# QizhiPei/FABind

Measured on AMD Instinct MI355X. Metric: complexes/sec fwd+bwd (1500p/40l nodes), full IaBNet on the whole graph (pocket model + 4-layer complex model + distance-map head on all nodes / pairs) with the pocket-cls + pocket-centre + coord + distmap + distmap-by-coords + distill losses (BASELINE configs[2] read literally), higher is better.
Workload: dtype bf16

## Files before the change

fabind_amd/_lib.py:

```python
import ctypes
import os

import torch

from . import config as _cfg

_HERE = os.path.dirname(os.path.abspath(__file__))
LIB_PATH = _cfg.knob("FABIND_LIB") or os.path.join(_HERE, "libfabind_hip.so")

ABI_VERSION = 19
DT_F32, DT_BF16 = 0, 1
ACT_NONE, ACT_SILU, ACT_RELU, ACT_SIGMOID, ACT_STORED_DERIV = 0, 1, 2, 3, 4
GEMM_FAM_NT_F32, GEMM_FAM_NT_F32_BF16, GEMM_FAM_NT_BF16, GEMM_FAM_GLDS, GEMM_FAM_PIPE, GEMM_FAM_X3, GEMM_FAM_X3_PRO, GEMM_FAM_PERSIST = range(8)

_vp, _i, _f, _l = ctypes.c_void_p, ctypes.c_int, ctypes.c_float, ctypes.c_long


class GemmArgs(ctypes.Structure):
    _fields_ = [(n, _vp) for n in ("A", "A2", "W", "C", "bias", "R", "r_index", "dotvec", "dot_out", "aux", "groups", "C2")] + \
               [(n, _i) for n in ("M", "N", "K", "K1", "lda", "lda2", "ldw", "ldc", "ldr", "ldaux", "dot_ld",
                                  "a_dtype", "w_dtype", "c_dtype", "aux_dtype", "act_pro", "act_epi", "dact_epi",
                                  "accumulate", "store_preact", "n_groups", "max_m", "max_n", "groups_ext", "epi_fast", "k_splits")] + \
               [("alpha", _f), ("p_drop", _f), ("drop_seed", ctypes.c_uint)] + \
               [(n, _vp) for n in ("row_mu", "row_rs", "col_c", "C16")] + [("ldc16", _i), ("split3", _i), ("r_dtype", _i), ("c2_bf16", _i)]
# ... 105 lines not shown
    "fabind_rowdot_bwd": [_vp, _i, _vp, _i, _vp, _i, _i, _i, _vp, _vp, _vp, _i, _vp],
    "fabind_edge_geom_bwd": [_vp, _vp, _vp, _vp, _vp, _vp, _vp, _vp, _vp, _vp, _i, _i, _i, _vp, _vp, _vp, _vp],
    "fabind_gcl_pre_bwd": [_vp, _i, _i, _vp, _vp, _i, _vp, _vp, _vp, _i, _vp],
    "fabind_gather_dact": [_vp, _i, _vp, _vp, _i, _i, _vp, _i, _i, _i, _vp],
    "fabind_coord_update_bwd": [_vp, _vp, _vp, _i, _i, _f, _vp, _vp, _vp, _vp],
    "fabind_cross_attn_bwd": [_vp, _i, _vp, _i, _vp, _i, _i, _i, _vp, _i, _i, _i, _f, _vp, _vp, _vp, _vp, _vp, _vp, _vp,
                              _vp, _vp, _vp],
    "fabind_pair_bias_cat": [_vp, _i, _vp, _i, _i, _i, _vp, _i, _vp, _i, _vp, _vp, _i, _vp, _i, _vp, _vp],
    "fabind_batched_transpose_pad": [_vp, _i, _vp, _i, _i, _i, _i, _vp, _vp],
    "fabind_node_chain_fwd": [_vp, _i, _vp, _i, _vp, _vp, _vp, _vp, _vp, _vp, _i, _i, _vp, _i, _vp, _i, _vp, _i, _i, _i, _vp],
    "fabind_node_chain_x3_fwd": [_vp, _i, _vp, _i, _vp, _vp, _vp, _vp, _vp, _vp, _vp, _vp, _vp, _vp, _i, _i, _vp, _i, _vp, _i, _vp, _i, _vp, _i, _vp, _i,
                                 _i, _i, _vp],
    "fabind_rows_hadamard_bwd": [_vp, _i, _i, _vp, _i, _i, _vp, _vp, _vp, _i, _vp, _i, _vp],
    "fabind_pair_hadamard_bwd_grid": [_vp, _i, _i, _vp, _i, _i, _vp, _vp, _vp, _vp, _i, _vp, _i, _vp],
    "fabind_pair_hadamard_bwd_rows": [_vp, _i, _i, _vp, _i, _i, _vp, _i, _i, _vp, _vp, _vp, _vp, _i, _vp, _i, _vp, _i, _vp],
    "fabind_pair_hadamard_bwd": [_vp, _i, _i, _vp, _vp, _i, _i, _vp, _vp, _i, _i, _vp, _vp, _i, _vp, _vp, _i, _vp, _vp, _i,
                                 _vp],
    "fabind_inter_attn_bwd": [_vp, _i, _vp, _i, _i, _vp, _vp, _vp, _vp, _vp, _vp, _vp, _vp, _vp, _vp, _vp, _vp, _f, _i,
                              _vp, _vp, _vp, _vp, _vp, _vp, _vp, _vp, _vp, _vp, _i, _vp],
    "fabind_inter_attn_bwd_rows": [_vp, _i, _vp, _i, _i, _vp, _vp, _vp, _vp, _vp, _vp, _vp, _vp, _vp, _vp, _vp, _vp, _f, _i,
                                   _vp, _vp, _vp, _vp, _vp, _vp, _vp, _vp, _vp, _vp, _i, _vp, _i, _i, _vp],
    "fabind_las_step_bwd": [_vp, _vp, _vp, _vp, _vp, _vp, _vp, _vp, _i, _i, _f, _f, _vp, _vp, _vp],
    "fabind_pair_bias_bwd": [_vp, _i, _vp, _i, _i, _vp, _vp, _i, _i, _i, _vp, _vp, _vp, _vp, _vp],
    "fabind_pair_bias_btcat": [_vp, _i, _vp, _vp, _vp, _i, _i, _i, _vp, _i, _i, _vp],
    "fabind_pair_bias_finish": [_vp, _vp, _i, _i, _vp, _vp, _i, _vp, _vp, _l, _vp],
    "fabind_pack_frag_multi": [_vp, _vp, _i, _vp],
    "fabind_lower_bound": [_vp, _i, _vp, _i, _vp, _vp],
    "fabind_pocket_center_fwd": [_vp, _vp, _vp, _vp, _i, _i, _f, _i, _vp, _vp, _vp],
    "fabind_pocket_center_bwd": [_vp, _vp, _vp, _vp, _i, _i, _f, _vp, _vp, _vp, _vp, _vp],
    "fabind_pair_dist_fwd": [_vp, _i, _i, _vp, _vp, _f, _f, _f, _vp, _vp],
    "fabind_pair_dist_bwd": [_vp, _i, _i, _vp, _vp, _vp, _f, _f, _f, _vp, _vp, _vp],
    "fabind_block_hadamard_fwd": [_vp, _i, _i, _vp, _i, _vp, _i, _i, _vp, _i, _vp],
    "fabind_block_hadamard_bwd": [_vp, _i, _i, _vp, _i, _vp, _i, _vp, _i, _i, _vp, _i, _i, _vp, _vp, _i, _vp, _i, _vp],
    "fabind_loss_fwd": [_vp, _vp, _l, _vp, _vp, _vp, _l, _vp, _vp, _i, _vp, _l, _vp, _vp, _l, _f, _f, _f, _f, _f, _f, _vp, _vp, _vp, _vp, _vp, _vp],
    "fabind_loss_bwd": [_vp, _vp, _l, _vp, _vp, _vp, _l, _vp, _vp, _i, _l, _vp, _vp, _l, _f, _f, _f, _f, _f, _f, _vp, _vp, _vp,
                        _vp, _vp, _vp, _vp, _vp, _vp],
    "fabind_layernorm_fwd": [_vp, _vp, _vp, _f, _i, _i, _vp, _vp, _vp, _vp],
    "fabind_layernorm_bwd": [_vp, _vp, _vp, _vp, _vp, _i, _i, _vp, _vp, _vp, _vp],
}

_lib = None


def load():
    global _lib
    if _lib is not None:
        return _lib
    if not os.path.exists(LIB_PATH):
        raise RuntimeError(
            "fabind_amd: %s is missing -- build it with `python -m fabind_amd.build` (hipcc, gfx950). "
            "There is no CPU/eager fallback for the hot path." % LIB_PATH)
    lib = ctypes.CDLL(LIB_PATH)
    lib.fabind_last_error.restype = ctypes.c_char_p
    lib.fabind_abi_version.restype = ctypes.c_int
    got = lib.fabind_abi_version()
    if got != ABI_VERSION:
        raise RuntimeError("fabind_amd: %s has ABI version %d, this binding needs %d -- rebuild with `python -m fabind_amd.build`"
                           % (LIB_PATH, got, ABI_VERSION))
    lib.fabind_sizeof_args.argtypes, lib.fabind_sizeof_args.restype = [ctypes.c_int], ctypes.c_int
    lib.fabind_cross_attn_bwd_scratch.argtypes, lib.fabind_cross_attn_bwd_scratch.restype = [_i, _i, _i], ctypes.c_long
    lib.fabind_pair_bias_cat_parts.argtypes, lib.fabind_pair_bias_cat_parts.restype = [_i, _i], ctypes.c_long
    lib.fabind_cross_attn_fused_bwd_scratch.argtypes, lib.fabind_cross_attn_fused_bwd_scratch.restype = [_i, _i, _i, _i, _i], ctypes.c_long
    lib.fabind_cross_attn_fused_bwd_parts.argtypes, lib.fabind_cross_attn_fused_bwd_parts.restype = [_i, _i], ctypes.c_int
    lib.fabind_pair_bias_finish_parts.argtypes, lib.fabind_pair_bias_finish_parts.restype = [_i], ctypes.c_int
    lib.fabind_loss_blocks.argtypes, lib.fabind_loss_blocks.restype = [_l, _l, _l], ctypes.c_int
    for nm in ("fabind_pair_block_tile", "fabind_pair_block_chunk"):
# ... 58 lines not shown
```

fabind_amd/build.py:

```python
import os
import subprocess
import sys

HERE = os.path.dirname(os.path.abspath(__file__))
CSRC = os.path.join(HERE, "csrc")
INCLUDE = os.path.join(os.path.dirname(HERE), "include")
LIB = os.path.join(HERE, "libfabind_hip.so")
SOURCES = ["capi.hip", "gemm.hip", "graph.hip", "gcl.hip", "fused_edge.hip", "fused_edge_fwd2.hip", "fused_edge_fwd3.hip", "fused_edge_bwd3.hip", "fused_edge_bwd4.hip", "pair_fused.hip", "attn.hip", "inter_attn_rows.hip", "attn_mfma.hip", "norm.hip", "bwd.hip", "post_optim.hip", "node_chain.hip", "heads.hip", "symmetry.hip", "optim.hip", "ranking.hip"]
HIPCC = os.environ.get("HIPCC", "/opt/rocm/bin/hipcc")
FLAGS = ["--offload-arch=gfx950", "-O3", "-std=c++17", "-fPIC", "-Wno-comment", "-I" + INCLUDE, "-I" + CSRC]


def _stale(out, deps):
    if not os.path.exists(out):
        return True
    t = os.path.getmtime(out)
    return any(os.path.getmtime(d) > t for d in deps)


def build(force=False, verbose=True):
    objs = []
    hdrs = [os.path.join(CSRC, "common.h"), os.path.join(CSRC, "fused_common.h"), os.path.join(INCLUDE, "fabind_hip.h")]
    procs = []
    for src in SOURCES:
        sp = os.path.join(CSRC, src)
        if not os.path.exists(sp):
            raise RuntimeError("fabind_amd.build: source %s is missing" % sp)
        obj = os.path.join(CSRC, src.replace(".hip", ".o"))
        objs.append(obj)
        if force or _stale(obj, [sp] + hdrs):
            cmd = [HIPCC] + FLAGS + ["-c", sp, "-o", obj]
            if verbose:
                print(" ".join(cmd), flush=True)
            procs.append((src, subprocess.Popen(cmd)))
    for src, p in procs:
        if p.wait() != 0:
            raise RuntimeError("hipcc failed on " + src)
    if force or procs or _stale(LIB, objs):
        cmd = [HIPCC, "--offload-arch=gfx950", "-shared", "-fPIC", "-o", LIB] + objs
        if verbose:
            print(" ".join(cmd), flush=True)
        subprocess.check_call(cmd)
    return LIB


if __name__ == "__main__":
    build(force="--force" in sys.argv)
```

fabind_amd/csrc/heads.hip:

```cpp
#include "common.h"
#include "fabind_hip.h"

namespace {

constexpr int LOSS_THREADS = 256;
constexpr int LOSS_TERMS = 8;

__device__ __forceinline__ float agent_load(const float* p) { return __hip_atomic_load(p, __ATOMIC_RELAXED, __HIP_MEMORY_SCOPE_AGENT); }
__device__ __forceinline__ void agent_store(float* p, float v) { __hip_atomic_store(p, v, __ATOMIC_RELAXED, __HIP_MEMORY_SCOPE_AGENT); }

__device__ __forceinline__ float cls_target(const void* cls, int cls_dt, long i) {
    switch (cls_dt) {
        case 0: return ((const float*)cls)[i];
        case 1: return (float)((const long long*)cls)[i];
        case 2: return (float)((const int*)cls)[i];
        default: return (float)((const uint8_t*)cls)[i];
    }
}

__global__ __launch_bounds__(LOSS_THREADS) void loss_fwd_kernel(
    const float* __restrict__ coords, const float* __restrict__ coords_true, long n_coord, const float* __restrict__ y_pred,
    const float* __restrict__ y_by, const float* __restrict__ dis_map, long n_pair, const float* __restrict__ logits,
    const void* __restrict__ cls, int cls_dt, const uint8_t* __restrict__ mask, long n_cls, const float* __restrict__ center,
    const float* __restrict__ center_true, long n_center, float w_coord, float w_pair, float w_distill, float w_cls, float w_center,
    float delta, float* part, unsigned* ticket, float* out, float* loss_out, float* terms_out) {
    const long tid = (long)blockIdx.x * LOSS_THREADS + threadIdx.x, nthr = (long)gridDim.x * LOSS_THREADS;
    float acc[7] = {0.f, 0.f, 0.f, 0.f, 0.f, 0.f, 0.f};
    for (long i = tid; i < n_pair; i += nthr) {
        const float yp = y_pred[i], yb = y_by[i], dm = dis_map[i];
        const float a = yp - dm, b = yb - dm, c = yb - yp;
        acc[2] += a * a; acc[3] += b * b; acc[4] += c * c;
    }
    for (long i = tid; i < n_coord; i += nthr) {
        const float d = fabsf(coords[i] - coords_true[i]);
// ... 126 lines not shown
    const int lane = threadIdx.x & 63, wave = threadIdx.x >> 6;
#pragma unroll
    for (int k = 0; k < 4; ++k) {
        const float v = wave_sum(a[k]);
        if (lane == 0) sh[wave][k] = v;
    }
    __syncthreads();
    if (threadIdx.x == 0) {
        float t[4];
#pragma unroll
        for (int k = 0; k < 4; ++k) t[k] = ((sh[0][k] + sh[1][k]) + sh[2][k]) + sh[3][k];
        center[b * 3] = t[1] / t[0]; center[b * 3 + 1] = t[2] / t[0]; center[b * 3 + 2] = t[3] / t[0];
        wsum[b] = t[0];
    }
}

__global__ __launch_bounds__(256) void pocket_center_bwd_kernel(const float* __restrict__ logits, const uint8_t* __restrict__ mask,
                                                                const float* __restrict__ xyz, const float* __restrict__ noise,
                                                                int L, float inv_tau, const float* __restrict__ center,
                                                                const float* __restrict__ wsum, const float* __restrict__ dcenter,
                                                                long n, float* dlogits) {
    const long i = (long)blockIdx.x * 256 + threadIdx.x;
    if (i >= n) return;
    if (!mask[i]) { dlogits[i] = 0.f; return; }
    const int b = (int)(i / L);
    float ds;
    (void)pc_soft(logits[i], noise, i, inv_tau, &ds);
    const float dw = (dcenter[b * 3] * (xyz[i * 3] - center[b * 3]) + dcenter[b * 3 + 1] * (xyz[i * 3 + 1] - center[b * 3 + 1]) +
                      dcenter[b * 3 + 2] * (xyz[i * 3 + 2] - center[b * 3 + 2])) / wsum[b];
    dlogits[i] = dw * ds;
}


constexpr int PB_TP = 128;
constexpr int PB_CH = 20;

struct PairBlock { long pair_off; int P, C, p_row0, c_row0, tile0, pad; };

__device__ __forceinline__ int pb_find(const PairBlock* __restrict__ desc, int B, int tile) {
    int lo = 0, hi = B - 1;
    while (lo < hi) {
        const int mid = (lo + hi + 1) >> 1;
        if (desc[mid].tile0 <= tile) lo = mid; else hi = mid - 1;
    }
    return lo;
}

__global__ __launch_bounds__(256) void pair_dist_fwd_kernel(const PairBlock* __restrict__ desc, int B, const float* __restrict__ xp,
                                                            const float* __restrict__ xc, float scale, float lo, float hi, float* y) {
    const int b = pb_find(desc, B, blockIdx.x);
    const PairBlock d = desc[b];
    const int i0 = (blockIdx.x - d.tile0) * PB_TP, i1 = min(d.P, i0 + PB_TP);
    if (i0 >= d.P) return;
    const long n = (long)(i1 - i0) * d.C;
    for (long k = threadIdx.x; k < n; k += 256) {
        const int i = i0 + (int)(k / d.C), j = (int)(k % d.C);
        const float* a = xp + (size_t)(d.p_row0 + i) * 3;
        const float* c = xc + (size_t)(d.c_row0 + j) * 3;
        const float dx = a[0] - c[0], dy = a[1] - c[1], dz = a[2] - c[2];
        const float v = scale * sqrtf(dx * dx + dy * dy + dz * dz);
        y[d.pair_off + (long)i0 * d.C + k] = fminf(fmaxf(v, lo), hi);
    }
}

__global__ __launch_bounds__(256) void pair_dist_bwd_kernel(const PairBlock* __restrict__ desc, const float* __restrict__ xp,
                                                            const float* __restrict__ xc, const float* __restrict__ dy, float scale,
                                                            float lo, float hi, int max_C, float* part) {
    const int b = blockIdx.x, s = blockIdx.y;
    const PairBlock d = desc[b];
    __shared__ float sh[256][3];
    for (int j0 = 0; j0 < d.C; j0 += 256) {
        const int cw = min(256, d.C - j0);
        const int nl = 256 / cw, il = threadIdx.x / cw, j = j0 + threadIdx.x % cw;
        float ax = 0.f, ay = 0.f, az = 0.f;
        if (il < nl) {
            const float* c = xc + (size_t)(d.c_row0 + j) * 3;
            const float cx = c[0], cy = c[1], cz = c[2];
            for (int i = s + 8 * il; i < d.P; i += 8 * nl) {
                const float* a = xp + (size_t)(d.p_row0 + i) * 3;
// ... 79 lines not shown
                if (j < cw) *(float2*)(sm + ((size_t)il * PB_CH + j) * W + c2) = acc[j];
            __syncthreads();
            for (int k = threadIdx.x; k < cw * W; k += 256) {
                float v = 0.f;
                for (int l = 0; l < NL; ++l) v += sm[(size_t)l * PB_CH * W + k];
                po[k] = v;
            }
        }
    }
}
template <int W>
__global__ __launch_bounds__(256) void block_hadamard_fwd_kernel(const PairBlock* __restrict__ desc, int B, const float* __restrict__ tp,
                                                                 int ldtp, const float* __restrict__ tc, int ldtc, bf16_t* out, int ldo) {
    constexpr int CT = W / 8, RP = 256 / CT;
    const int b = pb_find(desc, B, blockIdx.x);
    const PairBlock d = desc[b];
    const int i0 = (blockIdx.x - d.tile0) * PB_TP, i1 = min(d.P, i0 + PB_TP);
    if (i0 >= d.P) return;
    const int ct = threadIdx.x % CT, rg = threadIdx.x / CT, c8 = ct * 8;
    for (int i = i0; i < i1; ++i) {
        const float4 p0 = *(const float4*)(tp + (size_t)(d.p_row0 + i) * ldtp + c8), p1 = *(const float4*)(tp + (size_t)(d.p_row0 + i) * ldtp + c8 + 4);
        bf16_t* orow = out + (size_t)(d.pair_off + (long)i * d.C) * ldo + c8;
        for (int j = rg; j < d.C; j += RP) {
            const float* c = tc + (size_t)(d.c_row0 + j) * ldtc + c8;
            const float4 q0 = *(const float4*)c, q1 = *(const float4*)(c + 4);
            typedef __attribute__((ext_vector_type(4))) unsigned int nc_u4;
            const nc_u4 v = {pack2_bf16(p0.x * q0.x, p0.y * q0.y), pack2_bf16(p0.z * q0.z, p0.w * q0.w),
                             pack2_bf16(p1.x * q1.x, p1.y * q1.y), pack2_bf16(p1.z * q1.z, p1.w * q1.w)};
            __builtin_nontemporal_store(v, (nc_u4*)(orow + (size_t)j * ldo));
        }
    }
}

__global__ __launch_bounds__(256) void block_hadamard_bwd_reduce_kernel(const PairBlock* __restrict__ desc, int B, const int* __restrict__ row_b,
                                                                        int W, int nchunk_max, const float* __restrict__ part, float* dtc,
                                                                        int lddc) {
    const int r = blockIdx.x, b = row_b[r];
    const PairBlock d = desc[b];
    const int j = r - d.c_row0, ch = j / PB_CH, jj = j % PB_CH;
    const int nt = (d.P + PB_TP - 1) / PB_TP;
    for (int c = threadIdx.x; c < W; c += 256) {
        float v = 0.f;
        for (int t = 0; t < nt; ++t) v += part[(((size_t)(d.tile0 + t) * nchunk_max + ch) * PB_CH + jj) * W + c];
        dtc[(size_t)r * lddc + c] = v;
    }
}

}

extern "C" int fabind_pair_block_tile(void) { return PB_TP; }
extern "C" int fabind_pair_block_chunk(void) { return PB_CH; }

extern "C" int fabind_pair_dist_fwd(const void* desc, int B, int n_tiles, const float* xp, const float* xc, float scale, float lo, float hi,
                                    float* y, hipStream_t stream) {
    if (B <= 0 || n_tiles <= 0) return 0;
    hipLaunchKernelGGL(pair_dist_fwd_kernel, dim3(n_tiles), dim3(256), 0, stream, (const PairBlock*)desc, B, xp, xc, scale, lo, hi, y);
    FB_CHECK_LAUNCH();
    return 0;
}
extern "C" int fabind_pair_dist_bwd(const void* desc, int B, int max_C, const float* xp, const float* xc, const float* dy, float scale,
                                    float lo, float hi, float* part, float* dxc, hipStream_t stream) {
    if (B <= 0) return 0;
    FB_REQUIRE(part && dxc && max_C > 0, "fabind_pair_dist_bwd: scratch [B][8][max_C][3] and the output are required");
    hipLaunchKernelGGL(pair_dist_bwd_kernel, dim3(B, 8), dim3(256), 0, stream, (const PairBlock*)desc, xp, xc, dy, scale, lo, hi, max_C, part);
    FB_CHECK_LAUNCH();
    hipLaunchKernelGGL(pair_dist_bwd_reduce_kernel, dim3(B), dim3(256), 0, stream, (const PairBlock*)desc, B, max_C, part, dxc);
    FB_CHECK_LAUNCH();
    return 0;
}
extern "C" int fabind_block_hadamard_fwd(const void* desc, int B, int n_tiles, const float* tp, int ldtp, const float* tc, int ldtc, int W,
                                         void* out, int ldo, hipStream_t stream) {
    FB_REQUIRE(W == 64 || W == 128 || W == 256 || W == 512, "fabind_block_hadamard_fwd: W in {64, 128, 256, 512}");
    FB_REQUIRE(ldtp % 4 == 0 && ldtc % 4 == 0 && ldo % 8 == 0 && ((((uintptr_t)tp | (uintptr_t)tc | (uintptr_t)out) & 15) == 0),
               "fabind_block_hadamard_fwd: 16-byte aligned rows");
    if (B <= 0 || n_tiles <= 0) return 0;
    const PairBlock* dd = (const PairBlock*)desc;
    bf16_t* o = (bf16_t*)out;
    if (W == 512) hipLaunchKernelGGL((block_hadamard_fwd_kernel<512>), dim3(n_tiles), dim3(256), 0, stream, dd, B, tp, ldtp, tc, ldtc, o, ldo);
    else if (W == 256) hipLaunchKernelGGL((block_hadamard_fwd_kernel<256>), dim3(n_tiles), dim3(256), 0, stream, dd, B, tp, ldtp, tc, ldtc, o, ldo);
    else if (W == 128) hipLaunchKernelGGL((block_hadamard_fwd_kernel<128>), dim3(n_tiles), dim3(256), 0, stream, dd, B, tp, ldtp, tc, ldtc, o, ldo);
// ... 90 lines not shown
```

fabind_amd/models/model.py:

```python
import random

import torch
import torch.nn as nn
import torch.nn.functional as F
from torch.nn import Linear

from .. import kernels as K
from .. import ops
from ..utils.utils import get_keepNode_tensor, gumbel_softmax_no_random
from .att_model import EfficientMCAttModel


class Transition_diff_out_dim(nn.Module):

    def __init__(self, embedding_channels=256, out_channels=256, n=4):
        super().__init__()
        self.layernorm = nn.LayerNorm(embedding_channels)
        self.linear1 = Linear(embedding_channels, n * embedding_channels)
        self.linear2 = Linear(n * embedding_channels, out_channels)
        torch.nn.init.xavier_uniform_(self.linear1.weight, gain=0.001)
        torch.nn.init.xavier_uniform_(self.linear2.weight, gain=0.001)

    def forward(self, z):
        shp = z.shape
# ... 252 lines not shown
        start = _offsets(reps)
        j = torch.arange(pi.shape[0], device=dev) - start[pi]
        ci = _offsets(ncnt)[pocket_batch][pi] + j
        kn = torch.stack([kcnt, ncnt]).tolist()
        return _Pairs(pi, ci, ops.PairBlocks(kn[0], kn[1], dev))

    def _complex_and_heads(self, data, g, plan=None):
        scale = self.coordinate_scale
        cb = data['compound'].batch
        if plan:
            Xn, Xl, cidx, pidx = plan['Xn'], plan['Xl'], plan['cidx'], plan['pidx']
        else:
            Xn = self.normalize_coord(g['X'].unsqueeze(-2)).float()
            Xl = self.normalize_coord(g['XL'].unsqueeze(-2)).float()
            seg1 = g['segment'].bool() if not g['segment'].is_floating_point() else g['segment'] > 0.5
            cidx = torch.nonzero(~seg1 & ~g['is_global']).squeeze(1)
            pidx = torch.nonzero(seg1 & ~g['is_global']).squeeze(1)
        Xo, Ho = self.complex_model(Xn, g['H'], batch_id=g['batch'], segment_id=g['segment'], mask=g['mask'],
                                    is_global=g['is_global'], compound_edge_index=g['c2c'], LAS_edge_index=g['LAS'],
                                    batched_complex_coord_LAS=Xl, LAS_mask=None)
        coords_n = ops.take_unique_rows(Xo, cidx).squeeze(-2)
        return Ho, cidx, pidx, coords_n

    def _dist_heads(self, data, g, Ho, cidx, pidx, coords_n):
        cb = data['compound'].batch
        pairs = g.get('pairs')
        if pairs is None:
            B = int(cb[-1].item()) + 1
            pairs = self._pair_lists(g['pocket_batch'], cb, torch.bincount(g['pocket_batch'], minlength=B), torch.bincount(cb, minlength=B))
        pi, ci = pairs
        ln = ops.layernorm(ops.take_unique_rows(Ho, torch.cat([pidx, cidx])), self.layernorm.weight, self.layernorm.bias, self.layernorm.eps)
        npk = pidx.shape[0]
        blocks = getattr(pairs, 'blocks', None)
        hd = ops.rows_hadamard(ln, pi, npk + ci, a_sorted=True, blocks=blocks, n_a=npk)
        wd = ops.mm_dtype()
        part = ops.linear_rowdot(hd, self.distmap_mlp[0].weight.to(wd), self.distmap_mlp[0].bias,
                                 self.distmap_mlp[2].weight[0].contiguous(), act_epi=K.ACT_RELU)
        y_pred = (part.sum(1) + self.distmap_mlp[2].bias).sigmoid() * 10
        xp = self.normalize_coord(g['pocket_xyz']).float()
        if blocks is not None and coords_n.is_cuda:
            y_by = ops.pair_dist(xp, coords_n, blocks, scale=self.coordinate_scale, lo=0.0, hi=10.0)
        else:
            y_by = self.unnormalize_coord((xp[pi] - ops.take_rows_few(coords_n, ci)).norm(dim=-1)).clamp(0, 10)
        return y_pred, y_by

    def forward(self, data, stage=1, train=False, plan=None):
        cb = data['compound'].batch
        if plan is not None:
            self._adopt_plan(plan, cb.device)
        if plan is not None:
            keep_idx = plan['keep_idx']
        else:
            keep_idx = torch.nonzero(data['pocket'].keepNode).squeeze(1) if (stage == 1 or self.pocket_pred_model.training) else None
        head = self._pocket_head(data, plan)
        training = self.pocket_pred_model.training
        center = self._soft_center(head['logits'], head['mask'], head['xyz'], noise=training)
        pocket_cls = torch.zeros_like(head['mask'], dtype=data.pocket_idx.dtype)
        pocket_cls[head['pb'], head['loc']] = data.pocket_idx
        if training:
            dist = torch.norm(data.coords_center - center, p=2, dim=-1).mean(dim=-1)
            final_stage = 2 if (dist < self.args.center_dist_threshold and random.random() < self.stage_prob) else 1
        else:
            final_stage = stage
        if final_stage == 2:
            c2 = center
            if self.args.local_eval or (self.args.train_pred_pocket_noise and train):
                c2 = center + self.args.train_pred_pocket_noise * (2 * torch.rand_like(center) - 1)
            g = self._stage2(data, head, c2)
        else:
            cx = data['complex']
# ... 63 lines not shown
```

fabind_amd/ops.py:

```python
import ctypes

import numpy as np
import torch

from . import config as _cfg
from . import kernels as K
from ._lib import GemmArgs, check, dt_code, load, ptr, stream


def act_dtype():
    return torch.float32 if _cfg.fp32_storage() else torch.bfloat16


mm_dtype = act_dtype


def needs_grad(*ts):
    return torch.is_grad_enabled() and any(torch.is_tensor(t) and t.requires_grad for t in ts)


_needs_grad = needs_grad


def _nchunk(rows):
# ... 1219 lines not shown
        check(load().fabind_pair_hadamard_bwd(ptr(dout), dt_code(dout.dtype), dout.stride(0), ptr(t), ptr(t), t.stride(0), W,
                                              None, None, 0, 0, ptr(ia), ptr(ib), ia.shape[0], ptr(dt_), ptr(dt_),
                                              dt_.stride(0), None, None, 0, stream()), "fabind_pair_hadamard_bwd")
        return dt_, None, None, None, None, None


def _rows_hadamard_csr(ia, ib, n, a_sorted=False):
    P = ia.shape[0]
    dev = ia.device
    ia64, ib64 = ia.long(), ib.long()
    pa = torch.arange(P, device=dev) if a_sorted else torch.argsort(ia64, stable=True)
    pb = torch.argsort(ib64, stable=True)
    one = torch.ones_like(ia64)
    ca = torch.zeros(n, dtype=torch.int64, device=dev).index_add_(0, ia64, one)
    cb_ = torch.zeros(n, dtype=torch.int64, device=dev).index_add_(0, ib64, one)
    rowptr = torch.zeros(n + 1, dtype=torch.int64, device=dev)
    rowptr[1:] = torch.cumsum(ca + cb_, 0)
    starts = rowptr[:-1]
    sa, sb = ia64[pa], ib64[pb]
    ar = torch.arange(P, device=dev)
    ra = ar - (torch.cumsum(ca, 0) - ca)[sa]
    rb = ar - (torch.cumsum(cb_, 0) - cb_)[sb]
    pair_idx = torch.empty(2 * P, dtype=torch.int32, device=dev)
    partner = torch.empty(2 * P, dtype=torch.int32, device=dev)
    posa, posb = starts[sa] + ra, starts[sb] + ca[sb] + rb
    pair_idx[posa], partner[posa] = pa.to(torch.int32), ib64[pa].to(torch.int32)
    pair_idx[posb], partner[posb] = pb.to(torch.int32), ia64[pb].to(torch.int32)
    return rowptr.to(torch.int32), pair_idx, partner


ROWS_HADAMARD_WALK = _cfg.knob("FABIND_ROWS_HADAMARD_WALK")


def _block_hadamard_fwd(t, bl, n_a):
    W = t.shape[1]
    if not (bl is not None and act_dtype() == torch.bfloat16 and t.dtype == torch.float32 and W in (64, 128, 256, 512) and t.stride(1) == 1
            and t.stride(0) % 4 == 0 and t.data_ptr() % 16 == 0 and n_a == bl.n_prows and t.shape[0] == bl.n_prows + bl.n_crows and n_a % 4 == 0):
        return None
    out = torch.empty((bl.n_pairs, W), dtype=torch.bfloat16, device=t.device)
    check(load().fabind_block_hadamard_fwd(bl.desc_ptr, bl.B, bl.n_tiles, ptr(t), t.stride(0), ptr(t[n_a:]), t.stride(0), W, ptr(out), W,
                                           stream()), "fabind_block_hadamard_fwd")
    return out


def rows_hadamard(t, idx_a, idx_b, a_sorted=False, blocks=None, n_a=0):
    ia, ib = idx_a.to(torch.int32).contiguous(), idx_b.to(torch.int32).contiguous()
    if _needs_grad(t):
        return _RowsHadamard.apply(t, ia, ib, a_sorted, blocks, n_a)
    fwd = _block_hadamard_fwd(t, blocks, n_a)
    if fwd is not None:
        return fwd
    dummy = t[:, :0]
    return K.pair_hadamard(t, t, dummy, dummy, ia, ib, act_dtype())


class _InterAttn(torch.autograd.Function):
    @staticmethod
    def forward(ctx, qkv, cv, h, x, d, rhohat, bias_part, w_rk, w_rv, wcr, w3, H, g, clampv, s_ext=None, Wc=None, bc=None, holder=None, Wc32=None):
        v_in = None
        if Wc is not None:
            c16 = getattr(qkv, "_fab_b16", None) if _cfg.get_precision() == "bf16" else None
            v_in = c16[1][:, 2 * H:] if (c16 is not None and c16[0] == qkv._version) else _mm_in(qkv[:, 2 * H:])
            if Wc32 is not None:
                cv, _ = K.gemm(qkv[:, 2 * H:], Wc32, bias=bc, force_x3=True)
            else:
                cv, _ = K.gemm(v_in, Wc, bias=bc)
        h16 = None
        if holder is not None:
            h16 = torch.empty((h.shape[0], H), dtype=torch.bfloat16, device=h.device)
            holder.append(h16)
        h_out, x_out, alpha, cvs = K.inter_attn_fwd(qkv, cv, H, h, x, d, rhohat, g.rp_int, g.col_int, g.red_idx,
                                                    bias_part, w_rk, w_rv, wcr, w3, clampv, s_ext, h16, deal=getattr(g, "int_deal", None))
        ctx.g, ctx.H, ctx.clampv, ctx.np = g, H, clampv, bias_part.shape[1]
        ctx.has_ext, ctx.has_cv = s_ext is not None, Wc is not None
        ctx.sink_h, ctx.Wct = _sink_of(h), (_stored_wt(Wc) if Wc is not None else None)
# ... 619 lines not shown
```

include/fabind_hip.h:

```cpp
#ifndef FABIND_HIP_H
#define FABIND_HIP_H

#include <stdint.h>

#ifdef __cplusplus
extern "C" {
#endif

#ifndef __HIP_PLATFORM_AMD__
typedef struct ihipStream_t* hipStream_t;
#endif

const char* fabind_last_error(void);
#define FABIND_ABI_VERSION 19
int fabind_abi_version(void);
int fabind_sizeof_args(int which);

typedef struct FabindGemmArgs {
    const void* A;
    const void* A2;
    const void* W;
    void* C;
    const float* bias;
    const void* R;
// ... 243 lines not shown
int fabind_las_step(const float* x, const float* x0, const int* las_i, const int* las_j, const int* las_off,
                    const int* node_off, const int* c_cnt, int B, int max_n, float step, float clampv, float* x_out,
                    unsigned char* pass_mask, hipStream_t stream);

int fabind_pocket_center_fwd(const float* logits, const uint8_t* mask, const float* xyz, const float* noise, int B, int L,
                             float tau, int hard, float* center, float* wsum, hipStream_t stream);
int fabind_pocket_center_bwd(const float* logits, const uint8_t* mask, const float* xyz, const float* noise, int B, int L,
                             float tau, const float* center, const float* wsum, const float* dcenter, float* dlogits,
                             hipStream_t stream);

int fabind_loss_blocks(long n_pair, long n_coord, long n_cls);
int fabind_loss_fwd(const float* coords, const float* coords_true, long n_coord, const float* y_pred, const float* y_by,
                    const float* dis_map, long n_pair, const float* logits, const void* cls, int cls_dt, const uint8_t* mask,
                    long n_cls, const float* center, const float* center_true, long n_center, float w_coord, float w_pair,
                    float w_distill, float w_cls, float w_center, float delta, float* part, unsigned* ticket, float* out,
                    float* loss_out, float* terms_out, hipStream_t stream);
int fabind_loss_bwd(const float* coords, const float* coords_true, long n_coord, const float* y_pred, const float* y_by,
                    const float* dis_map, long n_pair, const float* logits, const void* cls, int cls_dt, long n_cls,
                    const float* center, const float* center_true, long n_center, float w_coord, float w_pair, float w_distill,
                    float w_cls, float w_center, float delta, const float* fwd_out, const float* g_loss, const float* g_terms,
                    float* d_coords, float* d_y_pred, float* d_y_by, float* d_logits, float* d_center, hipStream_t stream);

int fabind_pair_block_tile(void);
int fabind_pair_block_chunk(void);
int fabind_pair_dist_fwd(const void* desc, int B, int n_tiles, const float* xp, const float* xc, float scale, float lo, float hi,
                         float* y, hipStream_t stream);
int fabind_pair_dist_bwd(const void* desc, int B, int max_C, const float* xp, const float* xc, const float* dy, float scale, float lo,
                         float hi, float* part, float* dxc, hipStream_t stream);
int fabind_block_hadamard_fwd(const void* desc, int B, int n_tiles, const float* tp, int ldtp, const float* tc, int ldtc, int W, void* out,
                              int ldo, hipStream_t stream);
int fabind_block_hadamard_bwd(const void* desc, int B, int n_tiles, const void* dout, int ldo, const float* tp, int ldtp,
                              const float* tc, int ldtc, int W, const int* row_b, int n_crows, int nchunk_max, float* part,
                              float* dtp, int lddp, float* dtc, int lddc, hipStream_t stream);

int fabind_select_rows(const float* x, const float* z, const uint8_t* mask, int n, int width, float* x_out,
                       hipStream_t stream);

int fabind_row_stats(const void* x, int x_dt, int ldx, float eps, int R, int C, float* mu, float* rs, hipStream_t stream);

int fabind_layernorm_rows(const void* x, int x_dt, int ldx, const float* w, const float* b, float eps, int R, int C, void* y,
                          int y_dt, int ldy, int pad_to, hipStream_t stream);
int fabind_edge_ln_concat(const float* h, int ldh, int H, const int* row, const int* col, const float* rhohat, const float* w,
                          const float* b, float eps, int E, void* y, int y_dt, int ldy, int pad_to, hipStream_t stream);

int fabind_edge_lnfold(const void* AB, int ldab, int Kp, int H, const int* row, const int* col, const float* rho,
                       const float* stat, float eps, const float* w_r, const float* c_r, const float* c_c, const float* dvec,
                       int E, void* out, float p_drop, unsigned seed, hipStream_t stream);
int fabind_edge_lnfold_bwd_blocks(int E);
int fabind_edge_lnfold_bwd(const void* AB, int ldab, int Kp, int H, const int* row, const int* col, const float* rho,
                           const float* stat, float eps, const float* w_r, const float* c_r, const float* c_c,
                           const void* out, const void* dout, int E, float p_drop, void* du, float* es,
                           float* drho, float* part, int n_blocks, hipStream_t stream);

int fabind_inter_coord_fold(const void* P, int ldp, int H, const int* col, const float* rho, const float* stat, float q_w,
                            float eps, const float* u, const float* d, const float* w3, int E, float* s_out, float p_drop,
                            unsigned seed, hipStream_t stream);
int fabind_layernorm_rows_bwd(const void* x, int x_dt, int ldx, const float* w, const void* dy, int dy_dt, int lddy, float eps,
                              int R, int C, void* dx, int dx_dt, int lddx, float* dw_part, float* db_part, int nblk, hipStream_t stream);
int fabind_edge_concat(const float* h, int ldh, int H, const int* row, const int* col, const float* rhohat, int E, void* y,
                       int y_dt, int ldy, int pad_to, hipStream_t stream);
int fabind_layernorm_fwd(const float* x, const float* w, const float* b, float eps, int R, int C, float* y, float* mean,
                         float* rstd, hipStream_t stream);
int fabind_layernorm_bwd(const float* x, const float* w, const float* dy, const float* mean, const float* rstd, int R,
                         int C, float* dx, float* dw_part, float* db_part, hipStream_t stream);

int fabind_add(const float* a, const float* b, float* out, long n, hipStream_t stream);
// ... 93 lines not shown
```

Measured before the change: 528.2.

## Fuse distance-map head backward: compute d(hadamard) in registers and reduce to row grads

```diff
diff --git a/fabind_amd/_lib.py b/fabind_amd/_lib.py
--- a/fabind_amd/_lib.py
+++ b/fabind_amd/_lib.py
@@ -161,6 +161,7 @@
     "fabind_pair_dist_bwd": [_vp, _i, _i, _vp, _vp, _vp, _f, _f, _f, _vp, _vp, _vp],
     "fabind_block_hadamard_fwd": [_vp, _i, _i, _vp, _i, _vp, _i, _i, _vp, _i, _vp],
     "fabind_block_hadamard_bwd": [_vp, _i, _i, _vp, _i, _vp, _i, _vp, _i, _i, _vp, _i, _i, _vp, _vp, _i, _vp, _i, _vp],
+    "fabind_distmap_dx": [_vp, _i, _i, _vp, _i, _i, _vp, _i, _vp, _i, _vp, _i, _vp, _i, _i, _vp, _vp, _i, _vp, _i, _vp],
     "fabind_loss_fwd": [_vp, _vp, _l, _vp, _vp, _vp, _l, _vp, _vp, _i, _vp, _l, _vp, _vp, _l, _f, _f, _f, _f, _f, _f, _vp, _vp, _vp, _vp, _vp, _vp],
     "fabind_loss_bwd": [_vp, _vp, _l, _vp, _vp, _vp, _l, _vp, _vp, _i, _l, _vp, _vp, _l, _f, _f, _f, _f, _f, _f, _vp, _vp, _vp,
                         _vp, _vp, _vp, _vp, _vp, _vp],
diff --git a/fabind_amd/build.py b/fabind_amd/build.py
--- a/fabind_amd/build.py
+++ b/fabind_amd/build.py
@@ -6,7 +6,7 @@
 CSRC = os.path.join(HERE, "csrc")
 INCLUDE = os.path.join(os.path.dirname(HERE), "include")
 LIB = os.path.join(HERE, "libfabind_hip.so")
-SOURCES = ["capi.hip", "gemm.hip", "graph.hip", "gcl.hip", "fused_edge.hip", "fused_edge_fwd2.hip", "fused_edge_fwd3.hip", "fused_edge_bwd3.hip", "fused_edge_bwd4.hip", "pair_fused.hip", "attn.hip", "inter_attn_rows.hip", "attn_mfma.hip", "norm.hip", "bwd.hip", "post_optim.hip", "node_chain.hip", "heads.hip", "symmetry.hip", "optim.hip", "ranking.hip"]
+SOURCES = ["capi.hip", "gemm.hip", "graph.hip", "gcl.hip", "fused_edge.hip", "fused_edge_fwd2.hip", "fused_edge_fwd3.hip", "fused_edge_bwd3.hip", "fused_edge_bwd4.hip", "pair_fused.hip", "attn.hip", "inter_attn_rows.hip", "attn_mfma.hip", "norm.hip", "bwd.hip", "post_optim.hip", "node_chain.hip", "heads.hip", "distmap.hip", "symmetry.hip", "optim.hip", "ranking.hip"]
 HIPCC = os.environ.get("HIPCC", "/opt/rocm/bin/hipcc")
 FLAGS = ["--offload-arch=gfx950", "-O3", "-std=c++17", "-fPIC", "-Wno-comment", "-I" + INCLUDE, "-I" + CSRC]
 
@@ -20,7 +20,7 @@
 
 def build(force=False, verbose=True):
     objs = []
-    hdrs = [os.path.join(CSRC, "common.h"), os.path.join(CSRC, "fused_common.h"), os.path.join(INCLUDE, "fabind_hip.h")]
+    hdrs = [os.path.join(CSRC, "common.h"), os.path.join(CSRC, "fused_common.h"), os.path.join(CSRC, "pair_block.h"), os.path.join(INCLUDE, "fabind_hip.h")]
     procs = []
     for src in SOURCES:
         sp = os.path.join(CSRC, src)
diff --git a/fabind_amd/csrc/distmap.hip b/fabind_amd/csrc/distmap.hip
--- /dev/null
+++ b/fabind_amd/csrc/distmap.hip
@@ -0,0 +1,194 @@
+#include "common.h"
+#include "fabind_hip.h"
+#include "pair_block.h"
+
+namespace {
+
+typedef __attribute__((address_space(1))) const void* gptr_t;
+typedef __attribute__((address_space(3))) void* lptr_t;
+
+template <int N> __device__ __forceinline__ void wait_vmcnt() { asm volatile("s_waitcnt vmcnt(%0)" ::"n"(N) : "memory"); }
+
+constexpr int DM_W = 512;
+constexpr int DM_BN = 128;
+static_assert(PB_TP == 128, "the row tile of distmap_dx_kernel is the pair blocks' protein tile");
+
+template <int BK_, int NSTAGE> __host__ __device__ constexpr size_t dm_lds_bytes() {
+    return (size_t)NSTAGE * (PB_TP + DM_BN) * BK_ * 2 + (size_t)NSTAGE * 2 * DM_BN * sizeof(float) + 2 * DM_BN * sizeof(float);
+}
+
+template <int BK_, int NSTAGE>
+__global__ __launch_bounds__(256, 2) void distmap_dx_kernel(const PairBlock* __restrict__ desc, int B, const bf16_t* __restrict__ dz, int lddz,
+                                                            int N, const bf16_t* __restrict__ Wt, int ldwt, const float* __restrict__ tp,
+                                                            int ldtp, const float* __restrict__ tc, int ldtc, float* dtp, int lddp,
+                                                            int part_rows, float* part) {
+    constexpr int ROWS = PB_TP + DM_BN;
+    constexpr int RPP = 1024 / (BK_ * 2);
+    constexpr int PT = ROWS / RPP, PPW = PT / 4;
+    constexpr int LPR = 64 / RPP;
+    static_assert(PPW * RPP == 64, "a wave stages rows of ONE operand");
+    extern __shared__ __attribute__((aligned(16))) unsigned char smem[];
+    bf16_t* sT = (bf16_t*)smem;
+    float* sTc = (float*)(smem + (size_t)NSTAGE * ROWS * BK_ * 2);
+    float* sRed = sTc + NSTAGE * 2 * DM_BN;
+
+    const int total = gridDim.x, L = blockIdx.x, q = total / 8, rr = total % 8, xcd = L % 8;
+    const int t = (xcd < rr ? xcd * (q + 1) : rr * (q + 1) + (xcd - rr) * q) + L / 8;
+    const int tile = t / (DM_W / DM_BN), n0 = (t % (DM_W / DM_BN)) * DM_BN;
+    const PairBlock d = desc[pb_find(desc, B, tile)];
+    const int i0 = (tile - d.tile0) * PB_TP;
+    if (i0 >= d.P) return;
+
+    const int tid = threadIdx.x, lane = tid & 63, wave = tid >> 6;
+    const int wm = wave >> 1, wn = wave & 1;
+    const int fr = lane & 15, fq = lane >> 4;
+    const int nk = N / BK_;
+    const int G = d.C * nk;
+
+    const bf16_t* src[PPW];
+#pragma unroll
+    for (int jp = 0; jp < PPW; ++jp) {
+        const int row = (wave * PPW + jp) * RPP + lane / LPR;
+        const int cl = lane % LPR;
+        const int chunk = (BK_ == 64) ? (cl ^ (row & 7)) : (cl ^ ((row >> 2) & 3));
+        if (row < PB_TP) {
+            const long gi = min(i0 + row, d.P - 1);
+            src[jp] = dz + (size_t)(d.pair_off + gi * d.C) * lddz + chunk * 8;
+        } else {
+            src[jp] = Wt + (size_t)(n0 + row - PB_TP) * ldwt + chunk * 8;
+        }
+    }
+    const long jstep = wave < 2 ? lddz : 0;
+    const float* src_tc = tc + (size_t)d.c_row0 * ldtc + n0 + wn * 64 + lane;
+    int s_g = 0, s_kt = 0;
+    long s_off = 0, s_tc = 0;
+    auto stage_next = [&]() {
+        bf16_t* base = sT + (size_t)(s_g % NSTAGE) * ROWS * BK_;
+#pragma unroll
+        for (int jp = 0; jp < PPW; ++jp)
+            __builtin_amdgcn_global_load_lds((gptr_t)(src[jp] + s_off + s_kt * BK_), (lptr_t)(base + (size_t)(wave * PPW + jp) * RPP * BK_), 16,
+                                             0, 0);
+        __builtin_amdgcn_global_load_lds((gptr_t)(src_tc + s_tc), (lptr_t)(sTc + ((s_g % NSTAGE) * 2 + wm) * DM_BN + wn * 64), 4, 0, 0);
+        ++s_g;
+        if (++s_kt == nk) { s_kt = 0; s_off += jstep; s_tc += ldtc; }
+    };
+
+    f32x4_t tpr[4][4], dacc[4][4], acc[4][4];
+#pragma unroll
+    for (int i = 0; i < 4; ++i)
+#pragma unroll
+        for (int jn = 0; jn < 4; ++jn) {
+#pragma unroll
+            for (int v = 0; v < 4; ++v) {
+                const int row = i0 + wm * 64 + i * 16 + fq * 4 + v;
+                const float x = tp[(size_t)(d.p_row0 + min(row, d.P - 1)) * ldtp + n0 + wn * 64 + jn * 16 + fr];
+                tpr[i][jn][v] = row < d.P ? x : 0.f;
+            }
+            dacc[i][jn] = f32x4_t{0.f, 0.f, 0.f, 0.f};
+            acc[i][jn] = f32x4_t{0.f, 0.f, 0.f, 0.f};
+        }
+
+#pragma unroll
+    for (int s = 0; s < NSTAGE - 1; ++s)
+        if (s_g < G) stage_next();
+
+    constexpr int OPS = PPW + 1;
+    int g = 0;
+    auto kstep = [&]() {
+        const int ahead = min(NSTAGE - 2, G - 1 - g);
+        if (ahead >= 2) wait_vmcnt<2 * OPS>(); else if (ahead == 1) wait_vmcnt<OPS>(); else wait_vmcnt<0>();
+        __builtin_amdgcn_s_barrier();
+        if (s_g < G) stage_next();
+        const bf16_t* tA = sT + (size_t)(g % NSTAGE) * ROWS * BK_;
+        const bf16_t* tB = tA + PB_TP * BK_;
+#pragma unroll
+        for (int kk = 0; kk < BK_ / 32; ++kk) {
+            bf16x8_t af[4], bfr[4];
+#pragma unroll
+            for (int i = 0; i < 4; ++i) {
+                const int ra = wm * 64 + i * 16 + fr, rb = wn * 64 + i * 16 + fr;
+                const int ca = (BK_ == 64) ? ((kk * 4 + fq) ^ (ra & 7)) : (fq ^ ((ra >> 2) & 3));
+                const int cb = (BK_ == 64) ? ((kk * 4 + fq) ^ (rb & 7)) : (fq ^ ((rb >> 2) & 3));
+                af[i] = *(const bf16x8_t*)&tA[ra * BK_ + ca * 8];
+                bfr[i] = *(const bf16x8_t*)&tB[rb * BK_ + cb * 8];
+            }
+#pragma unroll
+            for (int i = 0; i < 4; ++i)
+#pragma unroll
+                for (int jn = 0; jn < 4; ++jn)
+                    acc[i][jn] = __builtin_amdgcn_mfma_f32_16x16x32_bf16(af[i], bfr[jn], acc[i][jn], 0, 0, 0);
+        }
+        ++g;
+    };
+
+    for (int j = 0; j < d.C; ++j) {
+        for (int kt = 0; kt < nk; ++kt) kstep();
+        float s[4], tcv[4];
+#pragma unroll
+        for (int jn = 0; jn < 4; ++jn) tcv[jn] = sTc[(((g - 1) % NSTAGE) * 2 + wm) * DM_BN + wn * 64 + jn * 16 + fr];
+#pragma unroll
+        for (int jn = 0; jn < 4; ++jn) {
+            float sj = 0.f;
+#pragma unroll
+            for (int i = 0; i < 4; ++i)
+#pragma unroll
+                for (int v = 0; v < 4; ++v) {
+                    const float a = acc[i][jn][v];
+                    dacc[i][jn][v] += a * tcv[jn];
+                    sj += a * tpr[i][jn][v];
+                }
+            sj += __shfl_xor(sj, 16, 64);
+            sj += __shfl_xor(sj, 32, 64);
+            s[jn] = sj;
+#pragma unroll
+            for (int i = 0; i < 4; ++i) acc[i][jn] = f32x4_t{0.f, 0.f, 0.f, 0.f};
+        }
+        if (fq == 0) {
+#pragma unroll
+            for (int jn = 0; jn < 4; ++jn) sRed[wm * DM_BN + wn * 64 + jn * 16 + fr] = s[jn];
+        }
+        asm volatile("s_waitcnt lgkmcnt(0)" ::: "memory");
+        __builtin_amdgcn_s_barrier();
+        if (tid < DM_BN) part[((size_t)tile * part_rows + j) * DM_W + n0 + tid] = sRed[tid] + sRed[DM_BN + tid];
+    }
+
+#pragma unroll
+    for (int i = 0; i < 4; ++i)
+#pragma unroll
+        for (int v = 0; v < 4; ++v) {
+            const int row = i0 + wm * 64 + i * 16 + fq * 4 + v;
+            if (row < d.P) {
+#pragma unroll
+                for (int jn = 0; jn < 4; ++jn) dtp[(size_t)(d.p_row0 + row) * lddp + n0 + wn * 64 + jn * 16 + fr] = dacc[i][jn][v];
+            }
+        }
+}
+
+}
+
+extern "C" int fabind_distmap_dx(const void* desc, int B, int n_tiles, const void* dz, int lddz, int N, const void* Wt, int ldwt,
+                                 const float* tp, int ldtp, const float* tc, int ldtc, const int* row_b, int n_crows, int nchunk_max,
+                                 float* part, float* dtp, int lddp, float* dtc, int lddc, hipStream_t stream) {
+    constexpr int BK_ = 32, NSTAGE = 4;
+    FB_REQUIRE(N >= BK_ && N % BK_ == 0, "fabind_distmap_dx: the contraction width must be a positive multiple of 32");
+    FB_REQUIRE(lddz >= N && ldwt >= N && lddz % 8 == 0 && ldwt % 8 == 0 && ((((uintptr_t)dz | (uintptr_t)Wt) & 15) == 0),
+               "fabind_distmap_dx: dz / W^T rows must be 16-byte aligned");
+    FB_REQUIRE(ldtp >= DM_W && ldtc >= DM_W && lddp >= DM_W && lddc >= DM_W, "fabind_distmap_dx: tp / tc / dtp / dtc rows are 512 wide");
+    FB_REQUIRE(part && dtp && (dtc || n_crows <= 0) && nchunk_max > 0, "fabind_distmap_dx: scratch [n_tiles][nchunk_max][chunk][512] and outputs are required");
+    if (B <= 0 || n_tiles <= 0) return 0;
+    const size_t lds = dm_lds_bytes<BK_, NSTAGE>();
+    static bool attr_set = false;
+    if (!attr_set) {
+        (void)hipFuncSetAttribute((const void*)distmap_dx_kernel<BK_, NSTAGE>, hipFuncAttributeMaxDynamicSharedMemorySize, (int)lds);
+        attr_set = true;
+    }
+    hipLaunchKernelGGL((distmap_dx_kernel<BK_, NSTAGE>), dim3(n_tiles * (DM_W / DM_BN)), dim3(256), lds, stream, (const PairBlock*)desc, B,
+                       (const bf16_t*)dz, lddz, N, (const bf16_t*)Wt, ldwt, tp, ldtp, tc, ldtc, dtp, lddp, nchunk_max * PB_CH, part);
+    FB_CHECK_LAUNCH();
+    if (n_crows > 0) {
+        hipLaunchKernelGGL(block_hadamard_bwd_reduce_kernel, dim3(n_crows), dim3(256), 0, stream, (const PairBlock*)desc, B, row_b, DM_W,
+                           nchunk_max, part, dtc, lddc);
+        FB_CHECK_LAUNCH();
+    }
+    return 0;
+}
diff --git a/fabind_amd/csrc/heads.hip b/fabind_amd/csrc/heads.hip
--- a/fabind_amd/csrc/heads.hip
+++ b/fabind_amd/csrc/heads.hip
@@ -1,5 +1,6 @@
 #include "common.h"
 #include "fabind_hip.h"
+#include "pair_block.h"
 
 namespace {
 
@@ -192,19 +193,6 @@
 }
 
 
-constexpr int PB_TP = 128;
-constexpr int PB_CH = 20;
-
-struct PairBlock { long pair_off; int P, C, p_row0, c_row0, tile0, pad; };
-
-__device__ __forceinline__ int pb_find(const PairBlock* __restrict__ desc, int B, int tile) {
-    int lo = 0, hi = B - 1;
-    while (lo < hi) {
-        const int mid = (lo + hi + 1) >> 1;
-        if (desc[mid].tile0 <= tile) lo = mid; else hi = mid - 1;
-    }
-    return lo;
-}
 
 __global__ __launch_bounds__(256) void pair_dist_fwd_kernel(const PairBlock* __restrict__ desc, int B, const float* __restrict__ xp,
                                                             const float* __restrict__ xc, float scale, float lo, float hi, float* y) {
@@ -350,20 +338,6 @@
     }
 }
 
-__global__ __launch_bounds__(256) void block_hadamard_bwd_reduce_kernel(const PairBlock* __restrict__ desc, int B, const int* __restrict__ row_b,
-                                                                        int W, int nchunk_max, const float* __restrict__ part, float* dtc,
-                                                                        int lddc) {
-    const int r = blockIdx.x, b = row_b[r];
-    const PairBlock d = desc[b];
-    const int j = r - d.c_row0, ch = j / PB_CH, jj = j % PB_CH;
-    const int nt = (d.P + PB_TP - 1) / PB_TP;
-    for (int c = threadIdx.x; c < W; c += 256) {
-        float v = 0.f;
-        for (int t = 0; t < nt; ++t) v += part[(((size_t)(d.tile0 + t) * nchunk_max + ch) * PB_CH + jj) * W + c];
-        dtc[(size_t)r * lddc + c] = v;
-    }
-}
-
 }
 
 extern "C" int fabind_pair_block_tile(void) { return PB_TP; }
diff --git a/fabind_amd/csrc/pair_block.h b/fabind_amd/csrc/pair_block.h
--- /dev/null
+++ b/fabind_amd/csrc/pair_block.h
@@ -0,0 +1,34 @@
+#pragma once
+#include "common.h"
+
+namespace {
+
+constexpr int PB_TP = 128;
+constexpr int PB_CH = 20;
+
+struct PairBlock { long pair_off; int P, C, p_row0, c_row0, tile0, pad; };
+
+__device__ __forceinline__ int pb_find(const PairBlock* __restrict__ desc, int B, int tile) {
+    int lo = 0, hi = B - 1;
+    while (lo < hi) {
+        const int mid = (lo + hi + 1) >> 1;
+        if (desc[mid].tile0 <= tile) lo = mid; else hi = mid - 1;
+    }
+    return lo;
+}
+
+__global__ __launch_bounds__(256) void block_hadamard_bwd_reduce_kernel(const PairBlock* __restrict__ desc, int B, const int* __restrict__ row_b,
+                                                                        int W, int nchunk_max, const float* __restrict__ part, float* dtc,
+                                                                        int lddc) {
+    const int r = blockIdx.x, b = row_b[r];
+    const PairBlock d = desc[b];
+    const int j = r - d.c_row0, ch = j / PB_CH, jj = j % PB_CH;
+    const int nt = (d.P + PB_TP - 1) / PB_TP;
+    for (int c = threadIdx.x; c < W; c += 256) {
+        float v = 0.f;
+        for (int t = 0; t < nt; ++t) v += part[(((size_t)(d.tile0 + t) * nchunk_max + ch) * PB_CH + jj) * W + c];
+        dtc[(size_t)r * lddc + c] = v;
+    }
+}
+
+}
diff --git a/fabind_amd/models/model.py b/fabind_amd/models/model.py
--- a/fabind_amd/models/model.py
+++ b/fabind_amd/models/model.py
@@ -308,10 +308,9 @@
         ln = ops.layernorm(ops.take_unique_rows(Ho, torch.cat([pidx, cidx])), self.layernorm.weight, self.layernorm.bias, self.layernorm.eps)
         npk = pidx.shape[0]
         blocks = getattr(pairs, 'blocks', None)
-        hd = ops.rows_hadamard(ln, pi, npk + ci, a_sorted=True, blocks=blocks, n_a=npk)
         wd = ops.mm_dtype()
-        part = ops.linear_rowdot(hd, self.distmap_mlp[0].weight.to(wd), self.distmap_mlp[0].bias,
-                                 self.distmap_mlp[2].weight[0].contiguous(), act_epi=K.ACT_RELU)
+        part = ops.hadamard_rowdot(ln, pi, npk + ci, self.distmap_mlp[0].weight.to(wd), self.distmap_mlp[0].bias,
+                                   self.distmap_mlp[2].weight[0].contiguous(), a_sorted=True, blocks=blocks, n_a=npk)
         y_pred = (part.sum(1) + self.distmap_mlp[2].bias).sigmoid() * 10
         xp = self.normalize_coord(g['pocket_xyz']).float()
         if blocks is not None and coords_n.is_cuda:
diff --git a/fabind_amd/ops.py b/fabind_amd/ops.py
--- a/fabind_amd/ops.py
+++ b/fabind_amd/ops.py
@@ -1275,15 +1275,69 @@
 ROWS_HADAMARD_WALK = _cfg.knob("FABIND_ROWS_HADAMARD_WALK")
 
 
-def _block_hadamard_fwd(t, bl, n_a):
+def _blocks_fit(t, bl, n_a):
+    return (bl is not None and act_dtype() == torch.bfloat16 and t.dtype == torch.float32 and t.shape[1] in (64, 128, 256, 512) and t.stride(1) == 1
+            and t.stride(0) % 4 == 0 and t.data_ptr() % 16 == 0 and n_a == bl.n_prows and t.shape[0] == bl.n_prows + bl.n_crows)
+
+
+def _block_hadamard_launch(t, bl, n_a):
     W = t.shape[1]
-    if not (bl is not None and act_dtype() == torch.bfloat16 and t.dtype == torch.float32 and W in (64, 128, 256, 512) and t.stride(1) == 1
-            and t.stride(0) % 4 == 0 and t.data_ptr() % 16 == 0 and n_a == bl.n_prows and t.shape[0] == bl.n_prows + bl.n_crows and n_a % 4 == 0):
-        return None
     out = torch.empty((bl.n_pairs, W), dtype=torch.bfloat16, device=t.device)
     check(load().fabind_block_hadamard_fwd(bl.desc_ptr, bl.B, bl.n_tiles, ptr(t), t.stride(0), ptr(t[n_a:]), t.stride(0), W, ptr(out), W,
                                            stream()), "fabind_block_hadamard_fwd")
     return out
+
+
+def _block_hadamard_fwd(t, bl, n_a):
+    if not (_blocks_fit(t, bl, n_a) and n_a % 4 == 0):
+        return None
+    return _block_hadamard_launch(t, bl, n_a)
+
+
+class _HadamardRowdot(torch.autograd.Function):
+
+    @staticmethod
+    def forward(ctx, t, W, b, u, blocks, n_a):
+        hd = _block_hadamard_launch(t, blocks, n_a)
+        z, part = _gemm_rowdot(hd, W, b, u, K.ACT_NONE, K.ACT_RELU, store=True)
+        ctx.blocks, ctx.n_a, ctx.Wt = blocks, n_a, _stored_wt(W)
+        ctx.save_for_backward(t, W, u, z, hd)
+        return part
+
+    @staticmethod
+    def backward(ctx, dpart):
+        t, W, u, z, hd = ctx.saved_tensors
+        dz, du = _rowdot_bwd(z, dpart.contiguous(), u, K.ACT_RELU)
+        dt_ = _distmap_dx(dz, _wt(ctx.Wt, W), t, ctx.blocks, ctx.n_a)
+        dW, db = _param_grads(dz, hd, None, W, True, True)
+        return dt_, dW, db, du, None, None
+
+
+def _distmap_dx(dz, Wt, t, bl, n_a):
+    M, N = dz.shape
+    dt_ = torch.empty_like(t)
+    part = torch.empty((bl.n_tiles, bl.nchunk_max, bl.chunk, DISTMAP_W), dtype=torch.float32, device=t.device)
+    tc, dtc = t[n_a:], dt_[n_a:]
+    nbytes = 2.0 * M * N + 8.0 * t.shape[0] * DISTMAP_W + 8.0 * part.numel()
+    K._profiled("fabind_distmap_dx pairs=%d N=%d (d hd = dz W in registers -> d tp, d tc)" % (M, N), 2.0 * M * N * DISTMAP_W,
+                lambda: check(load().fabind_distmap_dx(bl.desc_ptr, bl.B, bl.n_tiles, ptr(dz), dz.stride(0), N, ptr(Wt), Wt.stride(0), ptr(t),
+                                                       t.stride(0), ptr(tc), t.stride(0), bl.row_b_ptr, bl.n_crows, bl.nchunk_max, ptr(part),
+                                                       ptr(dt_), dt_.stride(0), ptr(dtc), dt_.stride(0), stream()), "fabind_distmap_dx"),
+                nbytes)
+    return dt_
+
+
+DISTMAP_W = 512
+
+
+def hadamard_rowdot(t, idx_a, idx_b, W, b, u, a_sorted=False, blocks=None, n_a=0, p_drop=0.0):
+    if (p_drop == 0.0 and blocks is not None and t.is_cuda and _needs_grad(t, W, b, u) and b is not None and W.dtype == torch.bfloat16
+            and t.shape[1] == DISTMAP_W and W.shape[1] == DISTMAP_W and W.shape[0] % 32 == 0 and W.shape[0] >= 32 and W.is_contiguous()
+            and _blocks_fit(t, blocks, n_a)):
+        K.tn_hook(W, b)
+        return _HadamardRowdot.apply(t, W, b, u, blocks, n_a)
+    hd = rows_hadamard(t, idx_a, idx_b, a_sorted=a_sorted, blocks=blocks, n_a=n_a)
+    return linear_rowdot(hd, W, b, u, act_epi=K.ACT_RELU, p_drop=p_drop)
 
 
 def rows_hadamard(t, idx_a, idx_b, a_sorted=False, blocks=None, n_a=0):
diff --git a/include/fabind_hip.h b/include/fabind_hip.h
--- a/include/fabind_hip.h
+++ b/include/fabind_hip.h
@@ -299,6 +299,9 @@
 int fabind_block_hadamard_bwd(const void* desc, int B, int n_tiles, const void* dout, int ldo, const float* tp, int ldtp,
                               const float* tc, int ldtc, int W, const int* row_b, int n_crows, int nchunk_max, float* part,
                               float* dtp, int lddp, float* dtc, int lddc, hipStream_t stream);
+int fabind_distmap_dx(const void* desc, int B, int n_tiles, const void* dz, int lddz, int N, const void* Wt, int ldwt, const float* tp,
+                      int ldtp, const float* tc, int ldtc, const int* row_b, int n_crows, int nchunk_max, float* part, float* dtp, int lddp,
+                      float* dtc, int lddc, hipStream_t stream);
 
 int fabind_select_rows(const float* x, const float* z, const uint8_t* mask, int n, int width, float* x_out,
                        hipStream_t stream);
```

Result: no change. 523.1 (-1.0%).
